# BichenWuUCB/squeezeDet

Measured on AMD Instinct MI355X. Metric: images/sec SqueezeDet 1242x375 inference, higher is better.
Workload: dtype f16; 1 GPU; squeezeDet fp16 inference, batch=32 per GPU, synthetic 1242x375 images (4 distinct batches in rotation), full hot path (forward + interpret_output + filter_prediction + filtered rows to pinned host memory), inputs resident in HBM; 2 batches in flight (consecutive steps alternate between 2 HIP streams); global_batch=32, parallelism=dp1 (independent image shards, no collective)

## Files before the change

### squeezedet_amd/csrc/chain.hip

```cpp
#include "conv_common.h"
#include "chain.h"
#include "filter_body.h"

namespace sqdet {

namespace {

constexpr int CROWS = 8, CCOLS = 16;
constexpr int CHP = (CROWS + 2) * (CCOLS + 2);
constexpr int CCHUNK = CHP * 64;
constexpr int STAGE_B = 12288;
constexpr int NIMG = 2;

struct ChainGeom {
  int nch, nsq, nb1, nb3, chain, base3, per3, nstages;
};

__host__ __device__ inline ChainGeom chain_geom(int s, int e1, int e3, int s2) {
  ChainGeom g;
  g.nch = (s * 2 + 63) / 64;
  g.nsq = s2 / 16;
  g.nb1 = e1 / 64;
  g.nb3 = e3 / 64;
  g.chain = s2 > 0 ? 1 : 0;
  g.base3 = g.nb1 * (1 + g.chain);
  g.per3 = 3 * g.nch + g.chain;
  g.nstages = g.base3 + g.nb3 * g.per3;
  return g;
}

struct ChainArgs {
  const void* sq_in;
  void* sq_out;
  void* y;
  const unsigned char* stream;
  const float *b1, *b3, *bs2;
  int N, H, W, S, E1, E3, S2;
  int tiles_x, tiles_y;
  int nb1, nb3, nstages;
  unsigned in_bytes, out_bytes, y_bytes;
  int per_xcd;
  ChainRide ride;
};

__device__ __forceinline__ void glds16(unsigned voff, const unsigned char* sbase, unsigned lds_dst) {
  asm volatile("s_mov_b32 m0, %2\n\ts_nop 0\n\tglobal_load_lds_dwordx4 %0, %1" ::"v"(voff), "s"(sbase), "s"(lds_dst) : "memory", "m0");
}

#ifdef SQDET_CHAIN_TIMELINE
__device__ unsigned long long g_chain_tl[4096 * 8];
#define CTL(k) do { ctl[k] = wall_clock64(); } while (0)
#else
#define CTL(k) do {} while (0)
#endif

template <int N>
__device__ __forceinline__ void vm_wait() {
  asm volatile("s_waitcnt vmcnt(%0)" ::"n"(N) : "memory");
}

__device__ __forceinline__ i32x4 pack8(const f32x4& a, const f32x4& b) {
  f16x8 h = {(f16)a[0], (f16)a[1], (f16)a[2], (f16)a[3], (f16)b[0], (f16)b[1], (f16)b[2], (f16)b[3]};
  return __builtin_bit_cast(i32x4, h);
}

__device__ __forceinline__ f32x4 relu4(f32x4 v) {
  v[0] = fmaxf(v[0], 0.f); v[1] = fmaxf(v[1], 0.f); v[2] = fmaxf(v[2], 0.f); v[3] = fmaxf(v[3], 0.f);
  return v;
}

template <int NCH, int NSQ, bool WY, int RING, int DBG = 0>
__global__ __launch_bounds__(512, 2) void fire_chain(ChainArgs a) {
  using T = f16;
  constexpr int LOOK = RING - 2;
  constexpr int TH = (NSQ + 1) / 2;
  extern __shared__ __attribute__((aligned(16))) unsigned char lds[];
  const int lane = threadIdx.x & 63;
  const int wave = __builtin_amdgcn_readfirstlane((int)(threadIdx.x >> 6));
  const int pg = wave & 3, h = wave >> 2;
  const int j = lane & 15, g = lane >> 4;
#ifdef SQDET_CHAIN_TIMELINE
  unsigned long long ctl[8] = {0, 0, 0, 0, 0, 0, 0, 0};
#endif
  CTL(0);

  if ((int)(blockIdx.x >> 3) >= a.per_xcd) {
    const int rider = (int)((blockIdx.x >> 3) - a.per_xcd) * 8 + (int)(blockIdx.x & 7);
    FastLds<512>& fs = *reinterpret_cast<FastLds<512>*>(lds);
    for (int im = rider; im < a.ride.nimg; im += a.ride.nriders) {
      filter_one_image<true, f16, 512>(a.ride.fa, a.ride.da, a.ride.img0 + im, fs);
      __syncthreads();
    }
    return;
  }
  int b = (int)((blockIdx.x & 7) * a.per_xcd + (blockIdx.x >> 3));
  const int npairs = (a.N + 1) >> 1;
  if (b >= npairs * a.tiles_x * a.tiles_y) return;
  const int tx = b % a.tiles_x; b /= a.tiles_x;
  const int ty = b % a.tiles_y;
  const int np = b / a.tiles_y;
  const int oy0 = ty * CROWS, ox0 = tx * CCOLS;

  unsigned char* ring = lds;
  unsigned char* stile = lds + RING * STAGE_B;
  unsigned char* xch = stile + NIMG * NCH * CCHUNK;
  float* bl = reinterpret_cast<float*>(xch + (NSQ > 0 ? 32768 : 0));
  const unsigned ring_addr = (unsigned)(uintptr_t)(__attribute__((address_space(3))) unsigned char*)ring;

  constexpr int NP = NCH * 4;
  constexpr int SIT = (NIMG * CHP * NP + 511) / 512;
  i32x4 sv[SIT];
  {
    const int s_pieces = a.S * 2 / 16;
    const __amdgpu_buffer_rsrc_t rin = __builtin_amdgcn_make_buffer_rsrc(const_cast<void*>(a.sq_in), 0, a.in_bytes, 0x00020000);
    constexpr unsigned OOB = 0xfffffff0u;
#pragma unroll
    for (int it = 0; it < SIT; ++it) {
      const int idx = it * 512 + (int)threadIdx.x;
      const int im = idx / (CHP * NP);
      const int rem = idx - im * (CHP * NP);
      const int P = rem / NP, q = rem - P * NP;
      const int r = P / (CCOLS + 2), c = P - r * (CCOLS + 2);
      const int iy = oy0 - 1 + r, ix = ox0 - 1 + c;
      const int n = np * 2 + im;
      const bool ok = idx < NIMG * CHP * NP && q < s_pieces && n < a.N && iy >= 0 && iy < a.H && ix >= 0 && ix < a.W;
      const unsigned off = ok ? (unsigned)((((n * a.H + iy) * a.W + ix) * a.S) * 2 + q * 16) : OOB;
      sv[it] = __builtin_amdgcn_raw_buffer_load_b128(rin, off, 0, 0);
    }
  }

  const unsigned voff1 = (unsigned)(wave * 1024 + lane * 16), voff2 = voff1 + 8192;
  const unsigned char* sp = a.stream;
  const unsigned m0_lo = ring_addr + (unsigned)wave * 1024;
  unsigned m0n = m0_lo;
  auto refill = [&]() {
    if constexpr (DBG >= 2) return;
    glds16(voff1, sp, m0n);
    if (h == 0) glds16(voff2, sp, m0n + 8192);
    sp += STAGE_B;
    m0n = m0n + STAGE_B == m0_lo + RING * STAGE_B ? m0_lo : m0n + STAGE_B;
  };
#pragma unroll
  for (int s = 0; s < LOOK; ++s) refill();
  CTL(1);

  {
#pragma unroll
    for (int it = 0; it < SIT; ++it) {
      const int idx = it * 512 + (int)threadIdx.x;
      const int im = idx / (CHP * NP);
      const int rem = idx - im * (CHP * NP);
      const int P = rem / NP, q = rem - P * NP;
      if (idx < NIMG * CHP * NP)
        *reinterpret_cast<i32x4*>(stile + (im * NCH + (q >> 2)) * CCHUNK + P * 64 + (((q & 3) ^ ((P >> 1) & 3)) << 4)) = sv[it];
    }
    const int nbias = a.E1 + a.E3 + a.S2;
    for (int i = threadIdx.x; i < nbias; i += 512)
      bl[i] = i < a.E1 ? a.b1[i] : (i < a.E1 + a.E3 ? a.b3[i - a.E1] : a.bs2[i - a.E1 - a.E3]);
  }
  __syncthreads();
  CTL(2);

  const int img = pg >> 1, r0 = (pg & 1) * 4;
  const unsigned char* simg = stile + img * NCH * CCHUNK;
  auto load_b = [&](int c, int rr, int dx) {
    const int P = (r0 + rr) * (CCOLS + 2) + j + dx;
    return *reinterpret_cast<const i32x4*>(simg + c * CCHUNK + P * 64 + ((g ^ ((P >> 1) & 3)) << 4));
  };
  unsigned cbo = 0, nbo = STAGE_B;
  auto lda = [&](unsigned bo, int f) {
    return *reinterpret_cast<const i32x4*>(ring + bo + f * 1024 + lane * 16);
  };
  int ks = 0, ep_ks = -100;
  auto sync = [&](bool lds_writes) {
    bool st = false;
    if constexpr (WY) { st = (ks - ep_ks) < LOOK; ++ks; }
    if constexpr (DBG < 1) {
      if (h == 0) { if (st) vm_wait<2 * (LOOK - 1) + 4>(); else vm_wait<2 * (LOOK - 1)>(); }
      else { if (st) vm_wait<(LOOK - 1) + 4>(); else vm_wait<(LOOK - 1)>(); }
    }
    if (lds_writes) asm volatile("s_waitcnt lgkmcnt(0)" ::: "memory");
    if constexpr (DBG < 3) __builtin_amdgcn_s_barrier();
    asm volatile("" ::: "memory");
  };
  auto next_buf = [&]() {
    cbo = nbo;
    nbo = nbo + STAGE_B == RING * STAGE_B ? 0 : nbo + STAGE_B;
  };

  f32x4 accs[TH > 0 ? TH : 1][4];
#pragma unroll
  for (int t = 0; t < (TH > 0 ? TH : 1); ++t)
#pragma unroll
    for (int m = 0; m < 4; ++m) accs[t][m] = f32x4{0.f, 0.f, 0.f, 0.f};

  const int ctot = a.E1 + a.E3;
  const __amdgpu_buffer_rsrc_t ry = __builtin_amdgcn_make_buffer_rsrc(a.y, 0, WY ? a.y_bytes : 0u, 0x00020000);
  const int n_img = np * 2 + img;
  const int ox = ox0 + j;
  const bool col_ok = ox < a.W && n_img < a.N;

  i32x4 an[2];
  sync(false);
  CTL(3);
  refill();
#pragma unroll
  for (int n = 0; n < 2; ++n) an[n] = lda(0, 2 * h + n);

  auto finish_block = [&](f32x4 (&acc)[4][2], int cc0) {
    i32x4 bf[4];
    {
      const f32x4 bias0 = *reinterpret_cast<const f32x4*>(bl + cc0 + h * 32 + g * 8);
      const f32x4 bias1 = *reinterpret_cast<const f32x4*>(bl + cc0 + h * 32 + g * 8 + 4);
#pragma unroll
      for (int m = 0; m < 4; ++m) bf[m] = pack8(relu4(acc[m][0] + bias0), relu4(acc[m][1] + bias1));
    }
    if (WY) {
#pragma unroll
      for (int m = 0; m < 4; ++m) {
        const int oy = oy0 + r0 + m;
        const bool ok = col_ok && oy < a.H;
        const unsigned off = ok ? (unsigned)((((n_img * a.H + oy) * a.W + ox) * ctot + cc0 + h * 32 + g * 8) * 2) : 0xfffffff0u;
        __builtin_amdgcn_raw_buffer_store_b128(bf[m], ry, off, 0, 0);
      }
      ep_ks = ks;
    }
    if constexpr (NSQ > 0) {
      i32x4 fr[2][TH];
#pragma unroll
      for (int u = 0; u < 2; ++u)
#pragma unroll
        for (int i = 0; i < TH; ++i) {
          const int t = min(h * TH + i, NSQ - 1);
          fr[u][i] = lda(cbo, u * NSQ + t);
        }
#pragma unroll
      for (int m = 0; m < 4; ++m)
        *reinterpret_cast<i32x4*>(xch + (wave * 4 + m) * 1024 + lane * 16) = bf[m];
      sync(true);
      i32x4 bx[2][4];
#pragma unroll
      for (int u = 0; u < 2; ++u)
#pragma unroll
        for (int m = 0; m < 4; ++m) bx[u][m] = *reinterpret_cast<const i32x4*>(xch + ((pg + 4 * u) * 4 + m) * 1024 + lane * 16);
#pragma unroll
      for (int n = 0; n < 2; ++n) an[n] = lda(nbo, 2 * h + n);
#pragma unroll
      for (int u = 0; u < 2; ++u) {
#pragma unroll
        for (int i = 0; i < TH; ++i) {
          if (NSQ % 2 == 0 || h * TH + i < NSQ) {
#pragma unroll
            for (int m = 0; m < 4; ++m) mma16<T>(accs[i][m], fr[u][i], bx[u][m]);
          }
          if (u == 0 && i == 0) refill();
        }
      }
      next_buf();
    }
  };

  {
    i32x4 b1f[NCH][4];
#pragma unroll
    for (int c = 0; c < NCH; ++c)
#pragma unroll
      for (int m = 0; m < 4; ++m) b1f[c][m] = load_b(c, m + 1, 1);
#pragma unroll 1
    for (int blk = 0; blk < a.nb1; ++blk) {
      f32x4 acc[4][2];
#pragma unroll
      for (int m = 0; m < 4; ++m)
#pragma unroll
        for (int n = 0; n < 2; ++n) acc[m][n] = f32x4{0.f, 0.f, 0.f, 0.f};
      i32x4 ac[2];
#pragma unroll
      for (int n = 0; n < 2; ++n) ac[n] = an[n];
#pragma unroll
      for (int c = 0; c < NCH; ++c) {
        i32x4 nx[2];
        if (c + 1 < NCH) {
#pragma unroll
          for (int n = 0; n < 2; ++n) nx[n] = lda(cbo, (c + 1) * 4 + 2 * h + n);
        } else {
          sync(false);
#pragma unroll
          for (int n = 0; n < 2; ++n) nx[n] = lda(nbo, 2 * h + n);
        }
#pragma unroll
        for (int m = 0; m < 4; ++m) {
#pragma unroll
          for (int n = 0; n < 2; ++n) mma16<T>(acc[m][n], ac[n], b1f[c][m]);
          if (c + 1 == NCH && m == 2 * h) refill();
        }
#pragma unroll
        for (int n = 0; n < 2; ++n) ac[n] = nx[n];
      }
#pragma unroll
      for (int n = 0; n < 2; ++n) an[n] = ac[n];
      next_buf();
      finish_block(acc, blk * 64);
    }
  }

  CTL(4);
  i32x4 B[6][3];
#pragma unroll
  for (int rr = 0; rr < 2; ++rr)
#pragma unroll
    for (int dx = 0; dx < 3; ++dx) B[rr][dx] = load_b(0, rr, dx);
#pragma unroll 1
  for (int blk = 0; blk < a.nb3; ++blk) {
    f32x4 acc[4][2];
#pragma unroll
    for (int m = 0; m < 4; ++m)
#pragma unroll
      for (int n = 0; n < 2; ++n) acc[m][n] = f32x4{0.f, 0.f, 0.f, 0.f};
    i32x4 ac[2];
#pragma unroll
    for (int n = 0; n < 2; ++n) ac[n] = an[n];
#pragma unroll
    for (int c = 0; c < NCH; ++c) {
#pragma unroll
      for (int dy = 0; dy < 3; ++dy) {
        if (DBG >= 4 && blk > 0) {
        } else if (dy == 0) {
#pragma unroll
          for (int rr = 2; rr < 5; ++rr)
#pragma unroll
            for (int dx = 0; dx < 3; ++dx) B[rr][dx] = load_b(c, rr, dx);
        } else if (dy == 1) {
#pragma unroll
          for (int dx = 0; dx < 3; ++dx) B[5][dx] = load_b(c, 5, dx);
        } else {
#pragma unroll
          for (int rr = 0; rr < 2; ++rr)
#pragma unroll
            for (int dx = 0; dx < 3; ++dx) B[rr][dx] = load_b((c + 1) % NCH, rr, dx);
        }
#pragma unroll
        for (int dx = 0; dx < 3; ++dx) {
          i32x4 nx[2];
          if (DBG >= 5 && blk > 0) {
            nx[0] = ac[1]; nx[1] = ac[0];
            if (dx == 2) sync(false);
          } else if (dx < 2) {
#pragma unroll
            for (int n = 0; n < 2; ++n) nx[n] = lda(cbo, (dx + 1) * 4 + 2 * h + n);
          } else {
            sync(false);
#pragma unroll
            for (int n = 0; n < 2; ++n) nx[n] = lda(nbo, 2 * h + n);
          }
#pragma unroll
          for (int m = 0; m < 4; ++m) {
#pragma unroll
            for (int n = 0; n < 2; ++n) mma16<T>(acc[m][n], ac[n], B[m + dy][dx]);
            if (dx == 2 && m == 2 * h) refill();
          }
#pragma unroll
          for (int n = 0; n < 2; ++n) ac[n] = nx[n];
        }
        next_buf();
      }
    }
#pragma unroll
    for (int n = 0; n < 2; ++n) an[n] = ac[n];
    if constexpr (DBG >= 6) {
#pragma unroll
      for (int m = 0; m < 4; ++m)
#pragma unroll
        for (int n = 0; n < 2; ++n) accs[0][m] += acc[m][n];
      next_buf();
    } else {
      finish_block(acc, a.E1 + blk * 64);
    }
  }
  CTL(5);
  vm_wait<0>();
  CTL(6);

  if constexpr (NSQ > 0) {
    T* so = reinterpret_cast<T*>(a.sq_out);
    const float* bs = bl + a.E1 + a.E3;
#pragma unroll
    for (int m = 0; m < 4; ++m) {
      const int oy = oy0 + r0 + m;
      if (col_ok && oy < a.H) {
        T* dst = so + ((size_t)(n_img * a.H + oy) * a.W + ox) * a.S2 + g * 4 * NSQ;
#pragma unroll
        for (int i = 0; i < TH; ++i) {
          const int t = h * TH + i;
          if (t < NSQ) {
            const f32x4 bias = *reinterpret_cast<const f32x4*>(bs + g * 4 * NSQ + t * 4);
            store4<T>(dst + t * 4, relu4(accs[i][m] + bias));
          }
        }
      }
    }
  }
#ifdef SQDET_CHAIN_TIMELINE
  CTL(7);
  if (threadIdx.x == 0 && blockIdx.x < 4096) {
#pragma unroll
    for (int k = 0; k < 8; ++k) g_chain_tl[(size_t)blockIdx.x * 8 + k] = ctl[k];
  }
#endif
}

__global__ void chain_pack_kernel(const float* __restrict__ w1, const float* __restrict__ w3, const float* __restrict__ ws2,
                                  f16* __restrict__ out, int S, int E1, int E3, int S2, ChainGeom gm, size_t total) {
  for (size_t idx = (size_t)blockIdx.x * blockDim.x + threadIdx.x; idx < total; idx += (size_t)gridDim.x * blockDim.x) {
    size_t t = idx;
    const int e = t % 8; t /= 8;
    const int lane = t % 64; t /= 64;
    const int tile = t % 4; t /= 4;
    const int slot = t % 3; t /= 3;
    const int stage = (int)t;
    const int i = lane & 15, g = lane >> 4;
    int kind, blk, r;
    int cc0 = 0;
    if (stage < gm.base3) {
      blk = stage / (1 + gm.chain);
      r = stage - blk * (1 + gm.chain);
      kind = r == 0 ? 0 : 2;
      cc0 = blk * 64;
    } else {
      const int k2 = stage - gm.base3;
      blk = k2 / gm.per3;
      r = k2 - blk * gm.per3;
      kind = r < 3 * gm.nch ? 1 : 2;
      cc0 = E1 + blk * 64;
    }
    const float* src = kind == 0 ? w1 : (kind == 1 ? w3 : ws2);
    if (!src) continue;
    float v = 0.f;
    if (kind == 2) {
      const int f = slot * 4 + tile;
      if (f < 2 * gm.nsq) {
        const int u = f / gm.nsq, tt = f - u * gm.nsq;
        const int co = (i >> 2) * 4 * gm.nsq + tt * 4 + (i & 3);
        const int ci = cc0 + u * 32 + g * 8 + e;
        v = ws2[(size_t)ci * S2 + co];
      }
    } else {
      const int co = blk * 64 + (tile >> 1) * 32 + (i >> 2) * 8 + (tile & 1) * 4 + (i & 3);
      if (kind == 0) {
        const int ci = slot * 32 + g * 8 + e;
        if (slot < gm.nch && ci < S) v = w1[(size_t)ci * E1 + co];
      } else {
        const int c = r / 3, dy = r - c * 3;
        const int ci = c * 32 + g * 8 + e;
        if (ci < S) v = w3[((size_t)(dy * 3 + slot) * S + ci) * E3 + co];
      }
    }
    out[idx] = (f16)v;
  }
}
// ... 196 lines not shown
      const float* bs = bl + a.E1 + a.E3;
#pragma unroll
      for (int m = 0; m < 4; ++m) {
        const int oy = oy0 + r0 + m;
        if (col_ok && oy < a.H) {
          T* dst = so + ((size_t)(n_img * a.H + oy) * a.W + ox) * a.S2 + g * 4 * NSQ;
#pragma unroll
          for (int tq = 0; tq < NSQ; ++tq) {
            const f32x4 bias = *reinterpret_cast<const f32x4*>(bs + g * 4 * NSQ + tq * 4);
            store4<T>(dst + tq * 4, relu4(accs[tq][m] + bias));
          }
        }
      }
    }
    __syncthreads();
  }
}

bool fire_chain_stream_shape(int s, int e1, int e3, int s2) {
  return s > 0 && s <= 32 && s % 8 == 0 && e1 % 64 == 0 && e3 % 64 == 0 && e1 > 0 && e3 > 0 && (s2 == 16 || s2 == 32 || s2 == 48) &&
         (size_t)((e1 / 64) * (4 + s2 / 8) + (e3 / 64) * (36 + s2 / 8)) * 1024 + CS_TILES * CS_TILE_B + (size_t)(e1 + e3 + s2) * 4 <= 160 * 1024;
}

template <int NSQ>
int launch_chain_stream(const ChainSArgs& a, hipStream_t st) {
  const size_t lds = (size_t)(a.nb1 * (4 + 2 * NSQ) + a.nb3 * (36 + 2 * NSQ)) * 1024 + CS_TILES * CS_TILE_B + (size_t)(a.E1 + a.E3 + a.S2) * 4;
  static PerDevice once;
  SQDET_CHECK_HIP(once.run([] { return hipFuncSetAttribute(reinterpret_cast<const void*>(&fire_chain_stream<NSQ>),
                                                           hipFuncAttributeMaxDynamicSharedMemorySize, 160 * 1024); }));
  int grid = cu_count();
  if (grid > (a.nquads + 7) / 8 * 8) grid = (a.nquads + 7) / 8 * 8;
  hipLaunchKernelGGL((fire_chain_stream<NSQ>), dim3((unsigned)grid), dim3(512), lds, st, a);
  SQDET_CHECK_HIP(hipGetLastError());
  return SQDET_OK;
}

constexpr size_t chain_lds_bytes(int nch, int nsq, int ring, int nbias) {
  return (size_t)ring * STAGE_B + (size_t)NIMG * nch * CCHUNK + (nsq > 0 ? 32768 : 0) + (size_t)nbias * 4;
}
constexpr int chain_ring(int nch, int nsq) { return chain_lds_bytes(nch, nsq, 6, 768 + 96) <= 160 * 1024 ? 6 : 4; }

template <int NCH, int NSQ, bool WY>
int launch_chain(const ChainArgs& a, hipStream_t st) {
  constexpr int RG = chain_ring(NCH, NSQ);
  const size_t lds = chain_lds_bytes(NCH, NSQ, RG, a.E1 + a.E3 + a.S2);
  static PerDevice once;
  SQDET_CHECK_HIP(once.run([] { return hipFuncSetAttribute(reinterpret_cast<const void*>(&fire_chain<NCH, NSQ, WY, RG>),
                                                           hipFuncAttributeMaxDynamicSharedMemorySize, 160 * 1024); }));
  const int wgs = ((a.N + 1) / 2) * a.tiles_x * a.tiles_y;
  ChainArgs& am = const_cast<ChainArgs&>(a);
  am.per_xcd = (wgs + 7) / 8;
  const int riders_per_xcd = a.ride.nimg > 0 ? (a.ride.nriders + 7) / 8 : 0;
  const dim3 grid((unsigned)(8 * (am.per_xcd + riders_per_xcd)));
  static_assert(sizeof(FastLds<512>) <= RG * STAGE_B, "the rider's state lives in the ring's LDS");
#ifdef SQDET_CHAIN_DBG
  if constexpr (NCH == 3 && NSQ == 6 && !WY) {
    const int d = tune(TUNE_DBG);
    static bool dbg_attr = false;
    if (!dbg_attr) {
      (void)hipFuncSetAttribute(reinterpret_cast<const void*>(&fire_chain<NCH, NSQ, WY, RG, 1>), hipFuncAttributeMaxDynamicSharedMemorySize, 160 * 1024);
      (void)hipFuncSetAttribute(reinterpret_cast<const void*>(&fire_chain<NCH, NSQ, WY, RG, 2>), hipFuncAttributeMaxDynamicSharedMemorySize, 160 * 1024);
      (void)hipFuncSetAttribute(reinterpret_cast<const void*>(&fire_chain<NCH, NSQ, WY, RG, 3>), hipFuncAttributeMaxDynamicSharedMemorySize, 160 * 1024);
      (void)hipFuncSetAttribute(reinterpret_cast<const void*>(&fire_chain<NCH, NSQ, WY, RG, 4>), hipFuncAttributeMaxDynamicSharedMemorySize, 160 * 1024);
      (void)hipFuncSetAttribute(reinterpret_cast<const void*>(&fire_chain<NCH, NSQ, WY, RG, 5>), hipFuncAttributeMaxDynamicSharedMemorySize, 160 * 1024);
      (void)hipFuncSetAttribute(reinterpret_cast<const void*>(&fire_chain<NCH, NSQ, WY, RG, 6>), hipFuncAttributeMaxDynamicSharedMemorySize, 160 * 1024);
      dbg_attr = true;
    }
    switch (d) {
      case 1: hipLaunchKernelGGL((fire_chain<NCH, NSQ, WY, RG, 1>), grid, dim3(512), lds, st, a); return SQDET_OK;
      case 2: hipLaunchKernelGGL((fire_chain<NCH, NSQ, WY, RG, 2>), grid, dim3(512), lds, st, a); return SQDET_OK;
      case 3: hipLaunchKernelGGL((fire_chain<NCH, NSQ, WY, RG, 3>), grid, dim3(512), lds, st, a); return SQDET_OK;
      case 4: hipLaunchKernelGGL((fire_chain<NCH, NSQ, WY, RG, 4>), grid, dim3(512), lds, st, a); return SQDET_OK;
      case 5: hipLaunchKernelGGL((fire_chain<NCH, NSQ, WY, RG, 5>), grid, dim3(512), lds, st, a); return SQDET_OK;
      case 6: hipLaunchKernelGGL((fire_chain<NCH, NSQ, WY, RG, 6>), grid, dim3(512), lds, st, a); return SQDET_OK;
      default: break;
    }
  }
#endif
  hipLaunchKernelGGL((fire_chain<NCH, NSQ, WY, RG>), grid, dim3(512), lds, st, a);
  SQDET_CHECK_HIP(hipGetLastError());
  return SQDET_OK;
}

template <int NCH, bool WY>
int dispatch_chain_nsq(const ChainArgs& a, int nsq, hipStream_t st) {
  if (nsq == 0) { if constexpr (WY) return launch_chain<NCH, 0, true>(a, st); }
  if constexpr (NCH == 1) {
    switch (nsq) {
      case 1: return launch_chain<NCH, 1, WY>(a, st);
      case 2: return launch_chain<NCH, 2, WY>(a, st);
      case 3: return launch_chain<NCH, 3, WY>(a, st);
      default: break;
    }
  } else {
    switch (nsq) {
      case 3: return launch_chain<NCH, 3, WY>(a, st);
      case 4: return launch_chain<NCH, 4, WY>(a, st);
      case 6: return launch_chain<NCH, 6, WY>(a, st);
      default: break;
    }
  }
  set_error("fire_chain: unsupported next-squeeze width");
  return SQDET_EUNSUPPORTED;
}

}

bool fire_chain_eligible(int s, int e1, int e3, int s2, int dtype) {
  if (dtype != SQDET_F16 || conv_algo() != 0) return false;
  if (s <= 0 || s % 8 != 0 || s > 96) return false;
  if (e1 <= 0 || e3 <= 0 || e1 % 64 != 0 || e3 % 64 != 0) return false;
  if (!(s2 == 0 || s2 == 16 || s2 == 32 || s2 == 48 || s2 == 64 || s2 == 96)) return false;
  const ChainGeom g = chain_geom(s, e1, e3, s2);
  if (g.nch < 1 || g.nch > 3) return false;
  if (g.nsq != 0 && (g.nch == 1 ? g.nsq > 3 : g.nsq < 3)) return false;
  if (e1 + e3 + s2 > 768 + 96) return false;
  return chain_lds_bytes(g.nch, g.nsq, chain_ring(g.nch, g.nsq), e1 + e3 + s2) <= 160 * 1024;
}

}

using namespace sqdet;

extern "C" size_t sqdet_fire_chain_stream_bytes(int s1x1, int e1x1, int e3x3, int next_s1x1, int dtype) {
  if (!fire_chain_eligible(s1x1, e1x1, e3x3, next_s1x1, dtype)) return 0;
  return (size_t)(chain_geom(s1x1, e1x1, e3x3, next_s1x1).nstages + 5) * STAGE_B;
}

extern "C" int sqdet_fire_chain_pack(const float* w_e1_hwio, const float* w_e3_hwio, const float* w_next_s_hwio,
                                     void* stream_buf, int s1x1, int e1x1, int e3x3, int next_s1x1, int dtype,
                                     sqdet_stream_t stream) {
  SQDET_REQUIRE(stream_buf, "fire_chain_pack: null stream buffer");
  SQDET_UNSUPPORTED(!fire_chain_eligible(s1x1, e1x1, e3x3, next_s1x1, dtype), "fire_chain_pack: shape/dtype not covered");
  const ChainGeom g = chain_geom(s1x1, e1x1, e3x3, next_s1x1);
  const size_t total = (size_t)g.nstages * STAGE_B / 2;
  const int blocks = (int)((total + 255) / 256 > 4096 ? 4096 : (total + 255) / 256);
  hipLaunchKernelGGL(chain_pack_kernel, dim3(blocks), dim3(256), 0, as_stream(stream), w_e1_hwio, w_e3_hwio,
                     next_s1x1 > 0 ? w_next_s_hwio : nullptr, (f16*)stream_buf, s1x1, e1x1, e3x3, next_s1x1, g, total);
  SQDET_CHECK_HIP(hipGetLastError());
  return SQDET_OK;
}

extern "C" int sqdet_fire_chain_fwd(const void* sq_in, const void* stream_buf, const float* b_e1, const float* b_e3,
                                    const float* b_next_s, void* y, void* sq_out, int n, int h, int w, int s1x1,
                                    int e1x1, int e3x3, int next_s1x1, int dtype, sqdet_stream_t stream) {
  return sqdet::fire_chain_launch_ride(sq_in, stream_buf, b_e1, b_e3, b_next_s, y, sq_out, n, h, w, s1x1, e1x1, e3x3, next_s1x1, dtype,
                                       nullptr, as_stream(stream));
}

int sqdet::fire_chain_idle_cus(int n, int h, int w, int s1x1, int e1x1, int e3x3, int next_s1x1, int dtype) {
  if (!fire_chain_eligible(s1x1, e1x1, e3x3, next_s1x1, dtype)) return 0;
  const ChainGeom g = chain_geom(s1x1, e1x1, e3x3, next_s1x1);
  const long px = (long)n * h * w;
  if (g.nch == 1 && px > 100000) return 0;
  const int wgs = ((n + 1) / 2) * ((w + CCOLS - 1) / CCOLS) * ((h + CROWS - 1) / CROWS);
  const int per = (wgs + 7) / 8;
  return per < 32 ? (32 - per) * 8 : 0;
}

int sqdet::fire_chain_launch_ride(const void* sq_in, const void* stream_buf, const float* b_e1, const float* b_e3,
                                  const float* b_next_s, void* y, void* sq_out, int n, int h, int w, int s1x1,
                                  int e1x1, int e3x3, int next_s1x1, int dtype, const ChainRide* ride, hipStream_t st_in) {
  const sqdet_stream_t stream = reinterpret_cast<sqdet_stream_t>(st_in);
  SQDET_REQUIRE(sq_in && stream_buf && b_e1 && b_e3, "fire_chain_fwd: null pointer");
  SQDET_REQUIRE(n > 0 && h > 0 && w > 0, "fire_chain_fwd: bad dims");
  SQDET_REQUIRE((next_s1x1 > 0) == (sq_out != nullptr) && (next_s1x1 == 0 || b_next_s), "fire_chain_fwd: sq_out / next_s1x1 mismatch");
  SQDET_REQUIRE(y || sq_out, "fire_chain_fwd: no output");
  SQDET_UNSUPPORTED(!fire_chain_eligible(s1x1, e1x1, e3x3, next_s1x1, dtype), "fire_chain_fwd: shape/dtype not covered");
  const long px = (long)n * h * w;
  SQDET_UNSUPPORTED(px * (e1x1 + e3x3) * 2 >= (1L << 31), "fire_chain_fwd: tensor too large for 32-bit offsets");
  const ChainGeom g = chain_geom(s1x1, e1x1, e3x3, next_s1x1);
  ChainArgs a;
  a.sq_in = sq_in; a.sq_out = sq_out; a.y = y; a.stream = reinterpret_cast<const unsigned char*>(stream_buf);
  a.b1 = b_e1; a.b3 = b_e3; a.bs2 = b_next_s;
  a.N = n; a.H = h; a.W = w; a.S = s1x1; a.E1 = e1x1; a.E3 = e3x3; a.S2 = next_s1x1;
  a.tiles_x = (w + CCOLS - 1) / CCOLS; a.tiles_y = (h + CROWS - 1) / CROWS;
  a.nb1 = g.nb1; a.nb3 = g.nb3; a.nstages = g.nstages;
  a.in_bytes = (unsigned)(px * s1x1 * 2);
  a.out_bytes = (unsigned)(px * next_s1x1 * 2);
  a.y_bytes = (unsigned)(px * (e1x1 + e3x3) * 2);
  a.per_xcd = 0;
  if (ride) a.ride = *ride; else { a.ride = ChainRide{}; a.ride.nimg = 0; a.ride.nriders = 0; a.ride.img0 = 0; }
  hipStream_t st = as_stream(stream);
  if (!y && g.nch == 1 && (px > 100000 || tune(TUNE_DBG) == 31) && fire_chain_stream_shape(s1x1, e1x1, e3x3, next_s1x1) && tune(TUNE_DBG) != 30) {
    SQDET_REQUIRE(a.ride.nimg == 0, "fire_chain: the persistent form carries no riders");
    ChainSArgs c;
    c.sq_in = sq_in; c.sq_out = sq_out; c.stream = a.stream; c.b1 = b_e1; c.b3 = b_e3; c.bs2 = b_next_s;
    c.N = n; c.H = h; c.W = w; c.S = s1x1; c.E1 = e1x1; c.E3 = e3x3; c.S2 = next_s1x1;
    c.tiles_x = a.tiles_x; c.tiles_y = a.tiles_y;
    const long nt = (long)n * a.tiles_x * a.tiles_y;
    c.ntiles = (int)nt; c.nquads = (int)((nt + CS_TILES - 1) / CS_TILES);
    c.nb1 = g.nb1; c.nb3 = g.nb3; c.in_bytes = a.in_bytes;
    switch (g.nsq) {
      case 1: return launch_chain_stream<1>(c, st);
      case 2: return launch_chain_stream<2>(c, st);
      case 3: return launch_chain_stream<3>(c, st);
      default: break;
    }
  }
  if (g.nch == 1) return y ? dispatch_chain_nsq<1, true>(a, g.nsq, st) : dispatch_chain_nsq<1, false>(a, g.nsq, st);
  if (g.nch == 2) return y ? dispatch_chain_nsq<2, true>(a, g.nsq, st) : dispatch_chain_nsq<2, false>(a, g.nsq, st);
  return y ? dispatch_chain_nsq<3, true>(a, g.nsq, st) : dispatch_chain_nsq<3, false>(a, g.nsq, st);
}

#ifdef SQDET_CHAIN_TIMELINE
extern "C" int sqdet_debug_chain_timeline(unsigned long long* host, int count) {
  return (int)hipMemcpyFromSymbol(host, HIP_SYMBOL(sqdet::g_chain_tl), sizeof(unsigned long long) * count);
}
#endif
```

### squeezedet_amd/ops.py

```python
import ctypes as C

import numpy as np
import torch

from . import _lib
from ._lib import check, dtype_code, lib, pad_code, stream_ptr


def _dev(t, name, dtype=None):
    if not isinstance(t, torch.Tensor) or not t.is_cuda:
        raise _lib.SqdetError("%s must be a CUDA(HIP) tensor -- there is no CPU path" % name)
    if dtype is not None and t.dtype != dtype:
        raise _lib.SqdetError("%s must be %s, got %s" % (name, dtype, t.dtype))
    if not t.is_contiguous():
        raise _lib.SqdetError("%s must be contiguous" % name)
    return C.c_void_p(t.data_ptr())


def _out_size(n, k, s, padding):
    return -(-n // s) if padding.upper() == "SAME" else (n - k) // s + 1


class PackedConv:

# ... 181 lines not shown


def fire_squeeze_next(x, p_s, b_s, p_e1, b_e1, p_e3, b_e3, p_next_s, b_next_s):
    n, h, w, cin = [int(v) for v in x.shape]
    so = torch.empty((n, h, w, p_next_s.cout), dtype=x.dtype, device=x.device)
    check(lib().sqdet_fire_squeeze_next_fwd(_dev(x, "x"), _dev(p_s.data, "w_s"), _dev(b_s, "b_s", torch.float32),
                                            _dev(p_e1.data, "w_e1"), _dev(b_e1, "b_e1", torch.float32),
                                            _dev(p_e3.data, "w_e3"), _dev(b_e3, "b_e3", torch.float32),
                                            _dev(p_next_s.data, "w_next_s"), _dev(b_next_s, "b_next_s", torch.float32), _dev(so, "sq_out"),
                                            n, h, w, cin, p_s.cout, p_e1.cout, p_e3.cout, p_next_s.cout, dtype_code(x.dtype), stream_ptr()),
          "sqdet_fire_squeeze_next_fwd")
    return so


def fire_expand_squeeze_next(sq_in, p_e1, b_e1, p_e3, b_e3, p_next_s, b_next_s, pool=False):
    n, h, w, s = [int(v) for v in sq_in.shape]
    shape = (n, -(-h // 2), -(-w // 2), p_next_s.cout) if pool else (n, h, w, p_next_s.cout)
    so = torch.empty(shape, dtype=sq_in.dtype, device=sq_in.device)
    check(lib().sqdet_fire_expand_squeeze_next_fwd(_dev(sq_in, "sq_in"), _dev(p_e1.data, "w_e1"), _dev(b_e1, "b_e1", torch.float32),
                                                   _dev(p_e3.data, "w_e3"), _dev(b_e3, "b_e3", torch.float32),
                                                   _dev(p_next_s.data, "w_next_s"), _dev(b_next_s, "b_next_s", torch.float32),
                                                   _dev(so, "sq_out"), n, h, w, s, p_e1.cout, p_e3.cout, p_next_s.cout, int(bool(pool)),
                                                   dtype_code(sq_in.dtype), stream_ptr()), "sqdet_fire_expand_squeeze_next_fwd")
    return so


class FireChainStream:

    def __init__(self, w_e1_hwio, w_e3_hwio, w_next_s_hwio=None, dtype=torch.float16):
        w1 = w_e1_hwio.detach().to(torch.float32).contiguous()
        w3 = w_e3_hwio.detach().to(torch.float32).contiguous()
        ws = w_next_s_hwio.detach().to(torch.float32).contiguous() if w_next_s_hwio is not None else None
        self.s, self.e1, self.e3 = int(w1.shape[2]), int(w1.shape[3]), int(w3.shape[3])
        self.s2 = int(ws.shape[3]) if ws is not None else 0
        if tuple(w1.shape[:2]) != (1, 1) or tuple(w3.shape[:3]) != (3, 3, self.s) or \
                (ws is not None and tuple(ws.shape[:3]) != (1, 1, self.e1 + self.e3)):
            raise _lib.SqdetError("FireChainStream: kernel shapes do not form expand1x1 / expand3x3 / next squeeze1x1")
        self.dtype = dtype
        code = dtype_code(dtype)
        nbytes = lib().sqdet_fire_chain_stream_bytes(self.s, self.e1, self.e3, self.s2, code)
        if nbytes == 0:
            raise _lib.SqdetError("fire chain kernel does not cover s=%d e1=%d e3=%d next_s=%d %s"
                                  % (self.s, self.e1, self.e3, self.s2, dtype))
        self.data = torch.empty(nbytes, dtype=torch.uint8, device=w1.device)
        check(lib().sqdet_fire_chain_pack(_dev(w1, "w_e1"), _dev(w3, "w_e3"), _dev(ws, "w_next_s") if ws is not None else None,
                                          _dev(self.data, "stream"), self.s, self.e1, self.e3, self.s2, code, stream_ptr()),
              "sqdet_fire_chain_pack")


def fire_chain_supported(s, e1, e3, next_s, dtype):
    return lib().sqdet_fire_chain_stream_bytes(int(s), int(e1), int(e3), int(next_s), dtype_code(dtype)) > 0


def fire_chain(sq_in, chain, b_e1, b_e3, b_next_s=None, want_y=False):
    n, h, w, s = [int(v) for v in sq_in.shape]
    if s != chain.s or sq_in.dtype != chain.dtype:
        raise _lib.SqdetError("fire_chain: input does not match the packed stream")
    y = torch.empty((n, h, w, chain.e1 + chain.e3), dtype=sq_in.dtype, device=sq_in.device) if (want_y or chain.s2 == 0) else None
    so = torch.empty((n, h, w, chain.s2), dtype=sq_in.dtype, device=sq_in.device) if chain.s2 > 0 else None
    check(lib().sqdet_fire_chain_fwd(_dev(sq_in, "sq_in"), _dev(chain.data, "stream"), _dev(b_e1, "b_e1", torch.float32),
                                     _dev(b_e3, "b_e3", torch.float32),
                                     _dev(b_next_s, "b_next_s", torch.float32) if chain.s2 > 0 else None,
                                     _dev(y, "y") if y is not None else None, _dev(so, "sq_out") if so is not None else None,
                                     n, h, w, chain.s, chain.e1, chain.e3, chain.s2, dtype_code(sq_in.dtype), stream_ptr()),
          "sqdet_fire_chain_fwd")
    return y, so


def interpret_output(preds, anchors_f32, classes, anchors_per_grid, img_w, img_h, exp_thresh=1.0,
                     with_class_probs=False, out=None):
    n, gh, gw, ch = [int(v) for v in preds.shape]
    if ch != anchors_per_grid * (classes + 5):
        raise _lib.SqdetError("interpret_output: %d channels != %d*(%d+5)" % (ch, anchors_per_grid, classes))
    A = gh * gw * anchors_per_grid
    if tuple(anchors_f32.shape) != (A, 4):
        raise _lib.SqdetError("interpret_output: anchors must be [%d,4]" % A)
    dev = preds.device
    if out is not None:
        boxes, probs, cls = out
        if tuple(boxes.shape) != (n, A, 4) or tuple(probs.shape) != (n, A) or tuple(cls.shape) != (n, A) or cls.dtype != torch.int64:
            raise _lib.SqdetError("interpret_output: out tensors must be [N,A,4] f32, [N,A] f32, [N,A] int64")
    else:
        boxes = torch.empty((n, A, 4), dtype=torch.float32, device=dev)
        probs = torch.empty((n, A), dtype=torch.float32, device=dev)
        cls = torch.empty((n, A), dtype=torch.int64, device=dev)
    pcp = torch.empty((n, A, classes), dtype=torch.float32, device=dev) if with_class_probs else None
    pconf = torch.empty((n, A), dtype=torch.float32, device=dev) if with_class_probs else None
    check(lib().sqdet_interpret_output(_dev(preds, "preds"), _dev(anchors_f32, "anchors", torch.float32),
                                       _dev(boxes, "boxes"), _dev(probs, "probs"), _dev(cls, "cls"),
                                       _dev(pcp, "pcp") if pcp is not None else None,
                                       _dev(pconf, "pconf") if pconf is not None else None,
                                       n, gh, gw, int(anchors_per_grid), int(classes), float(img_w), float(img_h),
                                       float(exp_thresh), dtype_code(preds.dtype), stream_ptr()),
          "sqdet_interpret_output")
    if with_class_probs:
        return boxes, probs, cls, pcp, pconf
    return boxes, probs, cls


def filter_prediction(boxes, probs, cls, classes, top_n, nms_thresh, prob_thresh, max_out=None, out=None):
    n, A = int(probs.shape[0]), int(probs.shape[1])
    use_topn = 0 < top_n < A
    if max_out is None:
        max_out = top_n if use_topn else min(A, 1024)
    dev = probs.device
    if out is not None:
        ob, op, oc, oi, cnt = out
        if tuple(ob.shape) != (n, max_out, 4) or tuple(op.shape) != (n, max_out) or tuple(cnt.shape) != (n,):
            raise _lib.SqdetError("filter_prediction: out tensors do not match [N,%d,...]" % max_out)
    else:
        ob = torch.empty((n, max_out, 4), dtype=torch.float32, device=dev)
        op = torch.empty((n, max_out), dtype=torch.float32, device=dev)
# ... 780 lines not shown
```

Measured before the change: 82750 images/s.

## Restructure fire-chain tile prologue loads, index math, and squeeze-output stores

Replaces the per-element integer divisions in workgroup and tile indexing with precomputed reciprocal multiplies. Reorganizes the input-tile gather so each half-block loads one image with hoisted offsets via inline-asm buffer loads, issues the bias loads early into registers, and waits only for those loads rather than for the ring prefetch. Squeeze outputs are written with wide buffer stores using out-of-bounds masking, and the final wait no longer drains all outstanding stores. It also adds optional preallocated output tensors to fire_chain. The main risk is that hand-tuned vmcnt counts and raw asm loads are fragile if the load ordering assumptions are wrong.

```diff
diff --git a/squeezedet_amd/csrc/chain.hip b/squeezedet_amd/csrc/chain.hip
--- a/squeezedet_amd/csrc/chain.hip
+++ b/squeezedet_amd/csrc/chain.hip
@@ -39,12 +39,33 @@
   int tiles_x, tiles_y;
   int nb1, nb3, nstages;
   unsigned in_bytes, out_bytes, y_bytes;
+  unsigned nwg, tiles_xy, inv_tiles_xy, inv_tiles_x;
   int per_xcd;
   ChainRide ride;
 };
 
 __device__ __forceinline__ void glds16(unsigned voff, const unsigned char* sbase, unsigned lds_dst) {
   asm volatile("s_mov_b32 m0, %2\n\ts_nop 0\n\tglobal_load_lds_dwordx4 %0, %1" ::"v"(voff), "s"(sbase), "s"(lds_dst) : "memory", "m0");
+}
+
+template <bool FIRST>
+__device__ __forceinline__ void tile_load16(i32x4& dst, unsigned voff, const i32x4& rsrc) {
+  if constexpr (FIRST) asm volatile("s_nop 4\n\tbuffer_load_dwordx4 %0, %1, %2, 0 offen" : "=v"(dst) : "v"(voff), "s"(rsrc) : "memory");
+  else asm volatile("buffer_load_dwordx4 %0, %1, %2, 0 offen" : "=v"(dst) : "v"(voff), "s"(rsrc) : "memory");
+}
+__device__ __forceinline__ void bias_load(float& dst, const float* p) {
+  asm volatile("global_load_dword %0, %1, off" : "=v"(dst) : "v"(p) : "memory");
+}
+template <int SIT>
+__device__ __forceinline__ void set_up_landed(i32x4 (&sv)[SIT], float (&bv)[2]) {
+#pragma unroll
+  for (int it = 0; it < SIT; ++it) asm volatile("" : "+v"(sv[it]));
+  asm volatile("" : "+v"(bv[0]), "+v"(bv[1]));
+}
+
+__device__ __forceinline__ unsigned chain_sdiv(unsigned n, unsigned d, unsigned inv) {
+  const unsigned q = __umulhi(n, inv);
+  return n - q * d >= d ? q + 1 : q;
 }
 
 #ifdef SQDET_CHAIN_TIMELINE
@@ -93,12 +114,12 @@
     }
     return;
   }
-  int b = (int)((blockIdx.x & 7) * a.per_xcd + (blockIdx.x >> 3));
-  const int npairs = (a.N + 1) >> 1;
-  if (b >= npairs * a.tiles_x * a.tiles_y) return;
-  const int tx = b % a.tiles_x; b /= a.tiles_x;
-  const int ty = b % a.tiles_y;
-  const int np = b / a.tiles_y;
+  const unsigned b = (blockIdx.x & 7) * (unsigned)a.per_xcd + (blockIdx.x >> 3);
+  if (b >= a.nwg) return;
+  const int np = (int)chain_sdiv(b, a.tiles_xy, a.inv_tiles_xy);
+  const unsigned bt = b - (unsigned)np * a.tiles_xy;
+  const int ty = (int)chain_sdiv(bt, (unsigned)a.tiles_x, a.inv_tiles_x);
+  const int tx = (int)(bt - (unsigned)ty * (unsigned)a.tiles_x);
   const int oy0 = ty * CROWS, ox0 = tx * CCOLS;
 
   unsigned char* ring = lds;
@@ -107,25 +128,43 @@
   float* bl = reinterpret_cast<float*>(xch + (NSQ > 0 ? 32768 : 0));
   const unsigned ring_addr = (unsigned)(uintptr_t)(__attribute__((address_space(3))) unsigned char*)ring;
 
-  constexpr int NP = NCH * 4;
-  constexpr int SIT = (NIMG * CHP * NP + 511) / 512;
+  constexpr int SIT = NCH * 3;
+  constexpr int YOUNG = DBG >= 2 ? 0 : LOOK;
+  const int tl = (int)(threadIdx.x & 255);
+  const int q4 = tl & 3, p0 = tl >> 2;
   i32x4 sv[SIT];
+  float bv[2];
   {
     const int s_pieces = a.S * 2 / 16;
-    const __amdgpu_buffer_rsrc_t rin = __builtin_amdgcn_make_buffer_rsrc(const_cast<void*>(a.sq_in), 0, a.in_bytes, 0x00020000);
+    const unsigned long long xaddr = (unsigned long long)(uintptr_t)a.sq_in;
+    const i32x4 rin = {(int)(unsigned)xaddr, (int)(unsigned)((xaddr >> 32) & 0xffffu), (int)a.in_bytes, 0x00020000};
     constexpr unsigned OOB = 0xfffffff0u;
-#pragma unroll
-    for (int it = 0; it < SIT; ++it) {
-      const int idx = it * 512 + (int)threadIdx.x;
-      const int im = idx / (CHP * NP);
-      const int rem = idx - im * (CHP * NP);
-      const int P = rem / NP, q = rem - P * NP;
-      const int r = P / (CCOLS + 2), c = P - r * (CCOLS + 2);
-      const int iy = oy0 - 1 + r, ix = ox0 - 1 + c;
-      const int n = np * 2 + im;
-      const bool ok = idx < NIMG * CHP * NP && q < s_pieces && n < a.N && iy >= 0 && iy < a.H && ix >= 0 && ix < a.W;
-      const unsigned off = ok ? (unsigned)((((n * a.H + iy) * a.W + ix) * a.S) * 2 + q * 16) : OOB;
-      sv[it] = __builtin_amdgcn_raw_buffer_load_b128(rin, off, 0, 0);
+    const int n = np * 2 + h;
+    const unsigned base = (unsigned)(((n * a.H + oy0 - 1) * a.W + ox0 - 1) * a.S * 2 + q4 * 16);
+    unsigned pof[3];
+    bool pok[3];
+#pragma unroll
+    for (int pi = 0; pi < 3; ++pi) {
+      const int P = p0 + 64 * pi;
+      const int r = (P * 3641) >> 16, c = P - r * (CCOLS + 2);
+      pok[pi] = P < CHP && n < a.N && (unsigned)(oy0 - 1 + r) < (unsigned)a.H && (unsigned)(ox0 - 1 + c) < (unsigned)a.W;
+      pof[pi] = base + (unsigned)((r * a.W + c) * a.S * 2);
+    }
+#pragma unroll
+    for (int cc = 0; cc < NCH; ++cc) {
+      const bool qok = cc * 4 + q4 < s_pieces;
+#pragma unroll
+      for (int pi = 0; pi < 3; ++pi) {
+        const unsigned off = pok[pi] && qok ? pof[pi] + cc * 64 : OOB;
+        if (cc == 0 && pi == 0) tile_load16<true>(sv[0], off, rin);
+        else tile_load16<false>(sv[cc * 3 + pi], off, rin);
+      }
+    }
+    const int nbias = a.E1 + a.E3 + a.S2;
+#pragma unroll
+    for (int k = 0; k < 2; ++k) {
+      const int i = min((int)threadIdx.x + 512 * k, nbias - 1);
+      bias_load(bv[k], i < a.E1 ? a.b1 + i : (i < a.E1 + a.E3 ? a.b3 + (i - a.E1) : a.bs2 + (i - a.E1 - a.E3)));
     }
   }
 
@@ -144,19 +183,22 @@
   for (int s = 0; s < LOOK; ++s) refill();
   CTL(1);
 
+  if (h == 0) vm_wait<2 * YOUNG>(); else vm_wait<YOUNG>();
+  set_up_landed(sv, bv);
   {
-#pragma unroll
-    for (int it = 0; it < SIT; ++it) {
-      const int idx = it * 512 + (int)threadIdx.x;
-      const int im = idx / (CHP * NP);
-      const int rem = idx - im * (CHP * NP);
-      const int P = rem / NP, q = rem - P * NP;
-      if (idx < NIMG * CHP * NP)
-        *reinterpret_cast<i32x4*>(stile + (im * NCH + (q >> 2)) * CCHUNK + P * 64 + (((q & 3) ^ ((P >> 1) & 3)) << 4)) = sv[it];
+    unsigned char* dst = stile + h * NCH * CCHUNK + p0 * 64 + ((q4 ^ ((p0 >> 1) & 3)) << 4);
+#pragma unroll
+    for (int cc = 0; cc < NCH; ++cc)
+#pragma unroll
+      for (int pi = 0; pi < 2; ++pi) *reinterpret_cast<i32x4*>(dst + cc * CCHUNK + pi * 4096) = sv[cc * 3 + pi];
+    if (p0 < CHP - 128) {
+#pragma unroll
+      for (int cc = 0; cc < NCH; ++cc) *reinterpret_cast<i32x4*>(dst + cc * CCHUNK + 2 * 4096) = sv[cc * 3 + 2];
     }
     const int nbias = a.E1 + a.E3 + a.S2;
-    for (int i = threadIdx.x; i < nbias; i += 512)
-      bl[i] = i < a.E1 ? a.b1[i] : (i < a.E1 + a.E3 ? a.b3[i - a.E1] : a.bs2[i - a.E1 - a.E3]);
+#pragma unroll
+    for (int k = 0; k < 2; ++k)
+      if ((int)threadIdx.x + 512 * k < nbias) bl[threadIdx.x + 512 * k] = bv[k];
   }
   __syncthreads();
   CTL(2);
@@ -377,28 +419,41 @@
     }
   }
   CTL(5);
-  vm_wait<0>();
+  constexpr int SQ_STORES = NSQ > 0 ? 4 * (TH == 3 ? 2 : 1) : 0;
+  if constexpr (NSQ == 0) vm_wait<0>();
+
+  if constexpr (NSQ > 0) {
+    static_assert(TH <= 3, "");
+    const __amdgpu_buffer_rsrc_t rso = __builtin_amdgcn_make_buffer_rsrc(a.sq_out, 0, a.out_bytes, 0x00020000);
+    const float* bs = bl + a.E1 + a.E3 + g * 4 * NSQ;
+    const int nt = h == 0 ? TH : NSQ - TH;
+    f32x4 bias[TH];
+#pragma unroll
+    for (int i = 0; i < TH; ++i) bias[i] = *reinterpret_cast<const f32x4*>(bs + min(h * TH + i, NSQ - 1) * 4);
+    const unsigned row_b = (unsigned)(a.W * a.S2 * 2);
+    const unsigned off0 = (unsigned)((((n_img * a.H + oy0 + r0) * a.W + ox) * a.S2 + g * 4 * NSQ + h * TH * 4) * 2);
+#pragma unroll
+    for (int m = 0; m < 4; ++m) {
+      const bool ok = col_ok && oy0 + r0 + m < a.H && nt > 0;
+      const unsigned off = ok ? off0 + m * row_b : 0xfffffff0u;
+      f16x4 o[TH];
+#pragma unroll
+      for (int i = 0; i < TH; ++i) {
+        const f32x4 v = relu4(accs[i][m] + bias[i]);
+        o[i] = f16x4{(T)v[0], (T)v[1], (T)v[2], (T)v[3]};
+      }
+      if constexpr (TH == 1) {
+        __builtin_amdgcn_raw_buffer_store_b64(__builtin_bit_cast(i32x2, o[0]), rso, off, 0, 0);
+      } else {
+        const f16x8 o01 = {o[0][0], o[0][1], o[0][2], o[0][3], o[1][0], o[1][1], o[1][2], o[1][3]};
+        if (NSQ % 2 == 0 || h == 0) __builtin_amdgcn_raw_buffer_store_b128(__builtin_bit_cast(i32x4, o01), rso, off, 0, 0);
+        else __builtin_amdgcn_raw_buffer_store_b64(__builtin_bit_cast(i32x2, o[0]), rso, off, 0, 0);
+        if constexpr (TH == 3) __builtin_amdgcn_raw_buffer_store_b64(__builtin_bit_cast(i32x2, o[2]), rso, ok ? off + 16 : 0xfffffff0u, 0, 0);
+      }
+    }
+    vm_wait<SQ_STORES>();
+  }
   CTL(6);
-
-  if constexpr (NSQ > 0) {
-    T* so = reinterpret_cast<T*>(a.sq_out);
-    const float* bs = bl + a.E1 + a.E3;
-#pragma unroll
-    for (int m = 0; m < 4; ++m) {
-      const int oy = oy0 + r0 + m;
-      if (col_ok && oy < a.H) {
-        T* dst = so + ((size_t)(n_img * a.H + oy) * a.W + ox) * a.S2 + g * 4 * NSQ;
-#pragma unroll
-        for (int i = 0; i < TH; ++i) {
-          const int t = h * TH + i;
-          if (t < NSQ) {
-            const f32x4 bias = *reinterpret_cast<const f32x4*>(bs + g * 4 * NSQ + t * 4);
-            store4<T>(dst + t * 4, relu4(accs[i][m] + bias));
-          }
-        }
-      }
-    }
-  }
 #ifdef SQDET_CHAIN_TIMELINE
   CTL(7);
   if (threadIdx.x == 0 && blockIdx.x < 4096) {
@@ -830,6 +885,10 @@
   a.N = n; a.H = h; a.W = w; a.S = s1x1; a.E1 = e1x1; a.E3 = e3x3; a.S2 = next_s1x1;
   a.tiles_x = (w + CCOLS - 1) / CCOLS; a.tiles_y = (h + CROWS - 1) / CROWS;
   a.nb1 = g.nb1; a.nb3 = g.nb3; a.nstages = g.nstages;
+  a.tiles_xy = (unsigned)(a.tiles_x * a.tiles_y);
+  a.nwg = (unsigned)((n + 1) / 2) * a.tiles_xy;
+  const auto inv32 = [](unsigned d) { const unsigned long long q = (1ull << 32) / d; return (unsigned)(q > 0xffffffffull ? 0xffffffffull : q); };
+  a.inv_tiles_xy = inv32(a.tiles_xy); a.inv_tiles_x = inv32((unsigned)a.tiles_x);
   a.in_bytes = (unsigned)(px * s1x1 * 2);
   a.out_bytes = (unsigned)(px * next_s1x1 * 2);
   a.y_bytes = (unsigned)(px * (e1x1 + e3x3) * 2);
diff --git a/squeezedet_amd/ops.py b/squeezedet_amd/ops.py
--- a/squeezedet_amd/ops.py
+++ b/squeezedet_amd/ops.py
@@ -257,12 +257,18 @@
     return lib().sqdet_fire_chain_stream_bytes(int(s), int(e1), int(e3), int(next_s), dtype_code(dtype)) > 0
 
 
-def fire_chain(sq_in, chain, b_e1, b_e3, b_next_s=None, want_y=False):
+def fire_chain(sq_in, chain, b_e1, b_e3, b_next_s=None, want_y=False, out_y=None, out_sq=None):
     n, h, w, s = [int(v) for v in sq_in.shape]
     if s != chain.s or sq_in.dtype != chain.dtype:
         raise _lib.SqdetError("fire_chain: input does not match the packed stream")
-    y = torch.empty((n, h, w, chain.e1 + chain.e3), dtype=sq_in.dtype, device=sq_in.device) if (want_y or chain.s2 == 0) else None
-    so = torch.empty((n, h, w, chain.s2), dtype=sq_in.dtype, device=sq_in.device) if chain.s2 > 0 else None
+    y = so = None
+    if want_y or chain.s2 == 0:
+        y = out_y if out_y is not None else torch.empty((n, h, w, chain.e1 + chain.e3), dtype=sq_in.dtype, device=sq_in.device)
+    if chain.s2 > 0:
+        so = out_sq if out_sq is not None else torch.empty((n, h, w, chain.s2), dtype=sq_in.dtype, device=sq_in.device)
+    for t, c, name in ((y, chain.e1 + chain.e3, "out_y"), (so, chain.s2, "out_sq")):
+        if t is not None and (tuple(t.shape) != (n, h, w, c) or t.dtype != sq_in.dtype or not t.is_contiguous()):
+            raise _lib.SqdetError("fire_chain: %s must be a contiguous [%d,%d,%d,%d] %s tensor" % (name, n, h, w, c, sq_in.dtype))
     check(lib().sqdet_fire_chain_fwd(_dev(sq_in, "sq_in"), _dev(chain.data, "stream"), _dev(b_e1, "b_e1", torch.float32),
                                      _dev(b_e3, "b_e3", torch.float32),
                                      _dev(b_next_s, "b_next_s", torch.float32) if chain.s2 > 0 else None,
```

After: 82450 images/s. Within noise of the previous version (-0.4%).

## Add dedicated producer wave to stream fire-chain weights into the LDS ring

Applied to the files above, without the earlier changes.

For most fire-chain variants, adds a ninth wave (576 threads) that alone issues all global-to-LDS weight stream loads and joins the consumer barriers, so the eight compute waves stop issuing refills and stop waiting on vmcnt. It also precomputes swizzled LDS offsets for the B-operand loads, interleaves the 3x3 B-tile loads with the dx loop, and reloads the 1x1 B fragments per block for NCH==3 to lower register pressure. The launch bounds hint changes to 3 workgroups per CU for producer variants. The risk is extra barrier participants, register limits under the new occupancy hint, and the producer wave running ahead or stalling the ring.

```diff
diff --git a/squeezedet_amd/csrc/chain.hip b/squeezedet_amd/csrc/chain.hip
--- a/squeezedet_amd/csrc/chain.hip
+++ b/squeezedet_amd/csrc/chain.hip
@@ -54,6 +54,8 @@
 #define CTL(k) do {} while (0)
 #endif
 
+constexpr bool chain_producer(int nch, int nsq, bool wy) { return !(nch == 3 && nsq == 3) && !(nch >= 2 && nsq == 6 && wy); }
+
 template <int N>
 __device__ __forceinline__ void vm_wait() {
   asm volatile("s_waitcnt vmcnt(%0)" ::"n"(N) : "memory");
@@ -70,8 +72,9 @@
 }
 
 template <int NCH, int NSQ, bool WY, int RING, int DBG = 0>
-__global__ __launch_bounds__(512, 2) void fire_chain(ChainArgs a) {
+__global__ __launch_bounds__(chain_producer(NCH, NSQ, WY) ? 576 : 512, chain_producer(NCH, NSQ, WY) ? 3 : 2) void fire_chain(ChainArgs a) {
   using T = f16;
+  constexpr bool PROD = chain_producer(NCH, NSQ, WY);
   constexpr int LOOK = RING - 2;
   constexpr int TH = (NSQ + 1) / 2;
   extern __shared__ __attribute__((aligned(16))) unsigned char lds[];
@@ -86,6 +89,7 @@
 
   if ((int)(blockIdx.x >> 3) >= a.per_xcd) {
     const int rider = (int)((blockIdx.x >> 3) - a.per_xcd) * 8 + (int)(blockIdx.x & 7);
+    if (PROD && wave == 8) return;
     FastLds<512>& fs = *reinterpret_cast<FastLds<512>*>(lds);
     for (int im = rider; im < a.ride.nimg; im += a.ride.nriders) {
       filter_one_image<true, f16, 512>(a.ride.fa, a.ride.da, a.ride.img0 + im, fs);
@@ -106,6 +110,45 @@
   unsigned char* xch = stile + NIMG * NCH * CCHUNK;
   float* bl = reinterpret_cast<float*>(xch + (NSQ > 0 ? 32768 : 0));
   const unsigned ring_addr = (unsigned)(uintptr_t)(__attribute__((address_space(3))) unsigned char*)ring;
+
+  if constexpr (PROD) {
+    if (wave == 8) {
+      unsigned voff[12];
+#pragma unroll
+      for (int p = 0; p < 12; ++p) voff[p] = (unsigned)(p * 1024 + lane * 16);
+      const unsigned char* sp = a.stream;
+      unsigned m0n = ring_addr;
+      auto issue = [&]() {
+        if constexpr (DBG >= 2) return;
+#pragma unroll
+        for (int p = 0; p < 12; ++p) glds16(voff[p], sp, m0n + (unsigned)p * 1024);
+        sp += STAGE_B;
+        m0n = m0n + STAGE_B == ring_addr + RING * STAGE_B ? ring_addr : m0n + STAGE_B;
+      };
+#pragma unroll
+      for (int s = 0; s < LOOK; ++s) issue();
+      CTL(1);
+      __builtin_amdgcn_s_barrier();
+#pragma unroll 1
+      for (int k = 0; k <= a.nstages; ++k) {
+        if constexpr (DBG < 1) vm_wait<12 * (LOOK - 1)>();
+        if constexpr (DBG < 3) __builtin_amdgcn_s_barrier();
+        asm volatile("" ::: "memory");
+#ifdef SQDET_CHAIN_TIMELINE
+        if (k == 0) CTL(3);
+#endif
+        issue();
+      }
+      vm_wait<0>();
+#ifdef SQDET_CHAIN_TIMELINE
+      if (lane == 0 && blockIdx.x < 4096) {
+        g_chain_tl[(size_t)blockIdx.x * 8 + 1] = ctl[1];
+        g_chain_tl[(size_t)blockIdx.x * 8 + 3] = ctl[3];
+      }
+#endif
+      return;
+    }
+  }
 
   constexpr int NP = NCH * 4;
   constexpr int SIT = (NIMG * CHP * NP + 511) / 512;
@@ -134,7 +177,7 @@
   const unsigned m0_lo = ring_addr + (unsigned)wave * 1024;
   unsigned m0n = m0_lo;
   auto refill = [&]() {
-    if constexpr (DBG >= 2) return;
+    if constexpr (PROD || DBG >= 2) return;
     glds16(voff1, sp, m0n);
     if (h == 0) glds16(voff2, sp, m0n + 8192);
     sp += STAGE_B;
@@ -163,9 +206,16 @@
 
   const int img = pg >> 1, r0 = (pg & 1) * 4;
   const unsigned char* simg = stile + img * NCH * CCHUNK;
+  const int Pb = r0 * (CCOLS + 2) + j;
+  unsigned bo0[4], bo1[4];
+#pragma unroll
+  for (int k = 0; k < 4; ++k) {
+    bo0[k] = (unsigned)(Pb * 64 + ((g ^ (((Pb >> 1) + k) & 3)) << 4));
+    bo1[k] = (unsigned)(Pb * 64 + ((g ^ (((Pb >> 1) + k + (j & 1)) & 3)) << 4));
+  }
   auto load_b = [&](int c, int rr, int dx) {
-    const int P = (r0 + rr) * (CCOLS + 2) + j + dx;
-    return *reinterpret_cast<const i32x4*>(simg + c * CCHUNK + P * 64 + ((g ^ ((P >> 1) & 3)) << 4));
+    const unsigned o = dx == 1 ? bo1[rr & 3] : bo0[(rr + (dx >> 1)) & 3];
+    return *reinterpret_cast<const i32x4*>(simg + o + (c * CCHUNK + (rr * (CCOLS + 2) + dx) * 64));
   };
   unsigned cbo = 0, nbo = STAGE_B;
   auto lda = [&](unsigned bo, int f) {
@@ -174,8 +224,8 @@
   int ks = 0, ep_ks = -100;
   auto sync = [&](bool lds_writes) {
     bool st = false;
-    if constexpr (WY) { st = (ks - ep_ks) < LOOK; ++ks; }
-    if constexpr (DBG < 1) {
+    if constexpr (WY && !PROD) { st = (ks - ep_ks) < LOOK; ++ks; }
+    if constexpr (DBG < 1 && !PROD) {
       if (h == 0) { if (st) vm_wait<2 * (LOOK - 1) + 4>(); else vm_wait<2 * (LOOK - 1)>(); }
       else { if (st) vm_wait<(LOOK - 1) + 4>(); else vm_wait<(LOOK - 1)>(); }
     }
@@ -261,13 +311,18 @@
   };
 
   {
+    constexpr bool B1_PER_BLOCK = PROD && NCH == 3 && NSQ > 0;
     i32x4 b1f[NCH][4];
-#pragma unroll
-    for (int c = 0; c < NCH; ++c)
-#pragma unroll
-      for (int m = 0; m < 4; ++m) b1f[c][m] = load_b(c, m + 1, 1);
+    auto load_b1f = [&]() {
+#pragma unroll
+      for (int c = 0; c < NCH; ++c)
+#pragma unroll
+        for (int m = 0; m < 4; ++m) b1f[c][m] = load_b(c, m + 1, 1);
+    };
+    if constexpr (!B1_PER_BLOCK) load_b1f();
 #pragma unroll 1
     for (int blk = 0; blk < a.nb1; ++blk) {
+      if constexpr (B1_PER_BLOCK) load_b1f();
       f32x4 acc[4][2];
 #pragma unroll
       for (int m = 0; m < 4; ++m)
@@ -323,23 +378,23 @@
     for (int c = 0; c < NCH; ++c) {
 #pragma unroll
       for (int dy = 0; dy < 3; ++dy) {
-        if (DBG >= 4 && blk > 0) {
-        } else if (dy == 0) {
-#pragma unroll
-          for (int rr = 2; rr < 5; ++rr)
+        const bool ldb = !(DBG >= 4 && blk > 0);
+        if (ldb && dy == 0) {
+#pragma unroll
+          for (int rr = 2; rr < 4; ++rr)
 #pragma unroll
             for (int dx = 0; dx < 3; ++dx) B[rr][dx] = load_b(c, rr, dx);
-        } else if (dy == 1) {
-#pragma unroll
-          for (int dx = 0; dx < 3; ++dx) B[5][dx] = load_b(c, 5, dx);
-        } else {
-#pragma unroll
-          for (int rr = 0; rr < 2; ++rr)
-#pragma unroll
-            for (int dx = 0; dx < 3; ++dx) B[rr][dx] = load_b((c + 1) % NCH, rr, dx);
         }
 #pragma unroll
         for (int dx = 0; dx < 3; ++dx) {
+          if (ldb) {
+            if (dy < 2) {
+              B[4 + dy][dx] = load_b(c, 4 + dy, dx);
+            } else {
+#pragma unroll
+              for (int rr = 0; rr < 2; ++rr) B[rr][dx] = load_b((c + 1) % NCH, rr, dx);
+            }
+          }
           i32x4 nx[2];
           if (DBG >= 5 && blk > 0) {
             nx[0] = ac[1]; nx[1] = ac[0];
@@ -377,7 +432,7 @@
     }
   }
   CTL(5);
-  vm_wait<0>();
+  if constexpr (!PROD) vm_wait<0>();
   CTL(6);
 
   if constexpr (NSQ > 0) {
@@ -403,7 +458,8 @@
   CTL(7);
   if (threadIdx.x == 0 && blockIdx.x < 4096) {
 #pragma unroll
-    for (int k = 0; k < 8; ++k) g_chain_tl[(size_t)blockIdx.x * 8 + k] = ctl[k];
+    for (int k = 0; k < 8; ++k)
+      if (!PROD || (k != 1 && k != 3)) g_chain_tl[(size_t)blockIdx.x * 8 + k] = ctl[k];
   }
 #endif
 }
@@ -706,6 +762,7 @@
   am.per_xcd = (wgs + 7) / 8;
   const int riders_per_xcd = a.ride.nimg > 0 ? (a.ride.nriders + 7) / 8 : 0;
   const dim3 grid((unsigned)(8 * (am.per_xcd + riders_per_xcd)));
+  const dim3 block(chain_producer(NCH, NSQ, WY) ? 576 : 512);
   static_assert(sizeof(FastLds<512>) <= RG * STAGE_B, "the rider's state lives in the ring's LDS");
 #ifdef SQDET_CHAIN_DBG
   if constexpr (NCH == 3 && NSQ == 6 && !WY) {
@@ -721,17 +778,17 @@
       dbg_attr = true;
     }
     switch (d) {
-      case 1: hipLaunchKernelGGL((fire_chain<NCH, NSQ, WY, RG, 1>), grid, dim3(512), lds, st, a); return SQDET_OK;
-      case 2: hipLaunchKernelGGL((fire_chain<NCH, NSQ, WY, RG, 2>), grid, dim3(512), lds, st, a); return SQDET_OK;
-      case 3: hipLaunchKernelGGL((fire_chain<NCH, NSQ, WY, RG, 3>), grid, dim3(512), lds, st, a); return SQDET_OK;
-      case 4: hipLaunchKernelGGL((fire_chain<NCH, NSQ, WY, RG, 4>), grid, dim3(512), lds, st, a); return SQDET_OK;
-      case 5: hipLaunchKernelGGL((fire_chain<NCH, NSQ, WY, RG, 5>), grid, dim3(512), lds, st, a); return SQDET_OK;
-      case 6: hipLaunchKernelGGL((fire_chain<NCH, NSQ, WY, RG, 6>), grid, dim3(512), lds, st, a); return SQDET_OK;
+      case 1: hipLaunchKernelGGL((fire_chain<NCH, NSQ, WY, RG, 1>), grid, block, lds, st, a); return SQDET_OK;
+      case 2: hipLaunchKernelGGL((fire_chain<NCH, NSQ, WY, RG, 2>), grid, block, lds, st, a); return SQDET_OK;
+      case 3: hipLaunchKernelGGL((fire_chain<NCH, NSQ, WY, RG, 3>), grid, block, lds, st, a); return SQDET_OK;
+      case 4: hipLaunchKernelGGL((fire_chain<NCH, NSQ, WY, RG, 4>), grid, block, lds, st, a); return SQDET_OK;
+      case 5: hipLaunchKernelGGL((fire_chain<NCH, NSQ, WY, RG, 5>), grid, block, lds, st, a); return SQDET_OK;
+      case 6: hipLaunchKernelGGL((fire_chain<NCH, NSQ, WY, RG, 6>), grid, block, lds, st, a); return SQDET_OK;
       default: break;
     }
   }
 #endif
-  hipLaunchKernelGGL((fire_chain<NCH, NSQ, WY, RG>), grid, dim3(512), lds, st, a);
+  hipLaunchKernelGGL((fire_chain<NCH, NSQ, WY, RG>), grid, block, lds, st, a);
   SQDET_CHECK_HIP(hipGetLastError());
   return SQDET_OK;
 }
```

Result: faster. 82920 images/s before, 84570 images/s after, median of 6 (+2.0%).
